# AHHHZ975/SLAM-Duckietown

Measured on AMD Instinct MI355X. Metric: EKF update steps/sec, higher is better.
Workload: dtype f64

## Files before the change

### slam-duckietown_amd/csrc/ekf_kernels.hip

```cpp
#include <algorithm>
#include <type_traits>

#include "ekf_device.h"

#include "ekf_devfn.h"
#include "ekf_host_plan.h"
#include "ekf_launch.h"

namespace ekf {

constexpr int PCS = CMAX + 2;
constexpr int RCH = 8;
constexpr int CPAD = (CMAX + RCH - 1) / RCH * RCH;
constexpr int WCS = KTOT + 1;

constexpr int SQ = (CMAX + 2) / 3;
struct StageRegs {
  double wv[SQ], vv[SQ];
};
__device__ __forceinline__ void stage_issue(StageRegs& R, __amdgpu_buffer_rsrc_t rsV, __amdgpu_buffer_rsrc_t rsW,
                                            int Cl, int c, int kb, int kofs, int ld, int wave, int lane) {
  const int kc = min(kofs + lane, kb - 1);
  const unsigned kW = (unsigned)(((kc >> 2) * (ld >> 4)) * 64 + (kc & 3) * 16) * 8u;
  const unsigned kV = (unsigned)(kc * ld) * 8u;
// ... 1187 lines not shown
  int cmax = Cl;
#pragma unroll
  for (int sh = 32; sh > 0; sh >>= 1) cmax = max(cmax, __shfl_xor(cmax, sh));
  const int kb = kbase;
  const PanelIdx t = panel_idx(P, V, W, mu_in, mu_out, ld, pstride, b, n, w0);
  if (w0 >= neff_eff) {
    if (wave == 0) panel_beyond_bound<MCAP>(t, kb);
    return;
  }
  if (tid < CC + 1) S.sC[tid] = Cl;
  if (kb > 0) {
    const __amdgpu_buffer_rsrc_t rsV = rs_rsrc(t.Vb), rsW = rs_rsrc(t.Wb);
    constexpr int Q = (CC + 3) / 4;
    const int k8 = (kb + 7) & ~7;
    for (int kofs = 0; kofs < kb; kofs += 64) {
      const int k = kofs + lane, kc = min(k, kb - 1);
      const unsigned kW = (unsigned)(((kc >> 2) * (ld >> 4)) * 64 + (kc & 3) * 16) * 8u;
      const unsigned kV = (unsigned)(kc * ld) * 8u;
      double wv[Q], vv[Q];
#pragma unroll
      for (int q = 0; q < Q; ++q) {
        const int a = wave + 4 * q;
        wv[q] = 0.0;
        vv[q] = 0.0;
        if (a < c) {
          const int row = __builtin_amdgcn_readlane(Cl, a);
          wv[q] = ldb8(rsW, kW, (unsigned)((row >> 4) * 64 + (row & 15)) * 8u);
          vv[q] = ldb8(rsV, kV, (unsigned)row * 8u);
        }
      }
#pragma unroll
      for (int q = 0; q < Q; ++q) {
        const int a = wave + 4 * q;
        if (a < CC && k < k8) {
          const bool live = a < c && k < kb;
          S.sF[0][a][k] = live ? wv[q] : 0.0;
          S.sF[1][a][k] = live ? vv[q] : 0.0;
        }
      }
    }
  }
  double X[CC];
  if (wave == 0) {
    int Crow[CC];
#pragma unroll
    for (int a = 0; a < CC; ++a) Crow[a] = __builtin_amdgcn_readlane(Cl, a);
    panel_base_gather<CC>(t, Crow, X);
  } else {
#pragma unroll
    for (int a = 0; a < CC; ++a) X[a] = 0.0;
  }
  __syncthreads();
  if (kb > 0) {
    const double* vlane = t.Vb + t.ii;
    const double* wlane = t.Wb + (long)(t.ii >> 4) * 64 + (t.ii & 15);
    auto gather_pending = [&](auto need_w_tag) {
      constexpr bool NEEDW = decltype(need_w_tag)::value;
      double v[8], w[8];
      pg_load<NEEDW>(vlane, wlane, ld, t.ld16, kb, 8 * wave, v, w);
      for (int k0 = 8 * wave; k0 < kb; k0 += 32) {
        double vn[8], wn[8];
        pg_load<NEEDW>(vlane, wlane, ld, t.ld16, kb, k0 + 32, vn, wn);
        pg_accumulate<CC>(X, v, w, S.sF, S.sC, k0, w0, t.ii);
#pragma unroll
        for (int u = 0; u < 8; ++u) {
          v[u] = vn[u];
          w[u] = wn[u];
        }
      }
    };
    if (cmax > w0) gather_pending(std::true_type{});
    else gather_pending(std::false_type{});
    if (wave > 0) {
#pragma unroll
      for (int a = 0; a < CC; ++a) SP.sPart[wave - 1][a][lane] = X[a];
    }
    __syncthreads();
    if (wave > 0) return;
#pragma unroll
    for (int a = 0; a < CC; ++a) {
      double x = X[a];
#pragma unroll
      for (int q = 0; q < 3; ++q) x += SP.sPart[q][a][lane];
      X[a] = x;
    }
  } else if (wave > 0) {
    return;
  }
  {
    unsigned got = 0;
    for (int spin = 0; spin < SPLIT_SPIN_LIMIT; ++spin) {
      got = __hip_atomic_load(ready + b, __ATOMIC_RELAXED, __HIP_MEMORY_SCOPE_AGENT);
      if (got == seq) break;
      __builtin_amdgcn_s_sleep(4);
    }
    if (got != seq) {
      if (lane == 0) atomicOr(flags + b, EKF_FLAG_INTERNAL);
      return;
    }
    __builtin_amdgcn_fence(__ATOMIC_ACQUIRE, "agent");
  }
  const SolveOut& o = out[b];
  {
    const double2* src = reinterpret_cast<const double2*>(o.it);
    double2* dst = reinterpret_cast<double2*>(S.sIt);
    constexpr int PER = (int)(sizeof(SolveIter) / 16), CNT = MCAP * PER, Q = (CNT + 63) / 64;
    const int count = m * PER;
    double2 t0[Q];
#pragma unroll
    for (int q = 0; q < Q; ++q) t0[q] = src[min(lane + q * 64, CNT - 1)];
#pragma unroll
    for (int q = 0; q < Q; ++q)
      if (lane + q * 64 < count) dst[lane + q * 64] = t0[q];
  }
  WAVE_LDS_SYNC();
  panels_finish<MCAP>(t, o, S.sIt, S.sC, X);
}

template <bool NT>
__device__ __forceinline__ double2 ld2(const double* a) {
  double2 r;
  if (NT) {
    r.x = __builtin_nontemporal_load(a);
    r.y = __builtin_nontemporal_load(a + 1);
  } else {
    r = *reinterpret_cast<const double2*>(a);
  }
  return r;
}
template <bool NT>
__device__ __forceinline__ void st2(double* a, double2 v) {
  if (NT) {
    __builtin_nontemporal_store(v.x, a);
    __builtin_nontemporal_store(v.y, a + 1);
  } else {
    *reinterpret_cast<double2*>(a) = v;
  }
}

constexpr int FTS = 80;

template <int NKTM, int NKL, bool NT>
__global__ __launch_bounds__(256, 2) void k_flush(double* __restrict__ P, const double* __restrict__ V,
                                                  const double* __restrict__ W,
                                                  const double* __restrict__ dacc,
                                                  const int* __restrict__ nact,
                                                  const SolveOut* __restrict__ so, int ld, long pstride,
                                                  int nkt, int rows_per_block, int gx) {
  __shared__ double tiles[4][16 * FTS];
  __shared__ double vlds[NKL > 0 ? 4 : 1][NKL > 0 ? NKL * 4 * 64 : 1];
  const int b = blockIdx.z;
  const int n = min(nact[b], so[b].neff);
  const int wave = __builtin_amdgcn_readfirstlane(threadIdx.x >> 6);
  const int lane = threadIdx.x & 63;
  int bx, by = 0;
  {
    const int total = gridDim.x;
    const int lin = blockIdx.x;
    const int q = total >> 3, r = total & 7, xcd = lin & 7, slot = lin >> 3;
    int rem = ((xcd < r) ? xcd * (q + 1) : r * (q + 1) + (xcd - r) * q) + slot;
    for (;; ++by) {
      const int cnt = gx - (by * rows_per_block) / 256;
      if (rem < cnt || cnt <= 0) break;
      rem -= cnt;
    }
    bx = (by * rows_per_block) / 256 + rem;
  }
  const int j0 = (bx * 4 + wave) * 64;
  const int i_begin = by * rows_per_block;
  const int i_lim = min(n, j0 + 64);
  if (j0 >= n || i_begin >= i_lim) return;
  const int i_end = min(i_lim, i_begin + rows_per_block);
  const int li = lane & 15, lq = lane >> 4;
  const int rr = lane >> 5, rc = (lane & 31) * 2;
  const int ld16 = ld >> 4;
  double* Pb = P + (long)b * pstride;
  const double* Vb = V + (long)b * KTOT * ld;
  const double* Wb = W + (long)b * KTOT * ld;
  double* T = tiles[wave];
  int nct = (n - j0 + 15) >> 4;
  if (nct > 4) nct = 4;

  double vf[NKTM][4];
#pragma unroll
  for (int t = 0; t < NKTM; ++t)
#pragma unroll
    for (int ct = 0; ct < 4; ++ct)
      vf[t][ct] = (t < nkt && ct < nct) ? Vb[(long)(4 * t + lq) * ld + j0 + ct * 16 + li] : 0.0;
  double* VL = vlds[NKL > 0 ? wave : 0];
  if (NKL > 0) {
    double tmp[NKL > 0 ? NKL * 4 : 1];
#pragma unroll
    for (int t = 0; t < NKL; ++t)
#pragma unroll
      for (int ct = 0; ct < 4; ++ct)
        tmp[t * 4 + ct] = Vb[(long)(4 * min(NKTM + t, nkt - 1) + lq) * ld + j0 + ct * 16 + li];
#pragma unroll
    for (int t = 0; t < NKL; ++t)
#pragma unroll
      for (int ct = 0; ct < 4; ++ct) VL[(t * 4 + ct) * 64 + lane] = (NKTM + t < nkt && ct < nct) ? tmp[t * 4 + ct] : 0.0;
    WAVE_SYNC();
  }

  double2 g[8];
  const int lds = p_lds(ld);
  double* Pj = Pb + p_col(ld, j0 + rc);
  auto gload = [&](int i0) {
#pragma unroll
    for (int q = 0; q < 8; ++q) g[q] = ld2<NT>(Pj + (long)(i0 + 2 * q + rr) * lds);
  };
  gload(i_begin);
  const int i_last = i_begin + ((i_end - 1 - i_begin) & ~15);
  constexpr int NKT_ALL = NKTM + NKL;
  constexpr bool EARLYW = NKTM >= 12;
  double wf[NKT_ALL];
  auto wload = [&](int i0) {
    const double* wsrc = Wb + (long)(i0 >> 4) * 64 + lane;
#pragma unroll
    for (int t = 0; t < NKT_ALL; ++t) wf[t] = wsrc[(long)min(t, nkt - 1) * ld16 * 64];
  };
  if (EARLYW) wload(i_begin);
  for (int i0 = i_begin; i0 < i_end; i0 += 16) {
    const int i_next = min(i0 + 16, i_last);
    if (!EARLYW) wload(i0);
#pragma unroll
    for (int q = 0; q < 8; ++q) *reinterpret_cast<double2*>(&T[(2 * q + rr) * FTS + rc]) = g[q];
    WAVE_SYNC();
    gload(i_next);
    double4_t acc[4];
#pragma unroll
    for (int ct = 0; ct < 4; ++ct)
#pragma unroll
      for (int r = 0; r < 4; ++r) acc[ct][r] = T[(lq + 4 * r) * FTS + ct * 16 + li];
    WAVE_SYNC();
#pragma unroll
    for (int t = 0; t < NKTM; ++t)
      if (t < nkt) {
#pragma unroll
        for (int ct = 0; ct < 4; ++ct)
          acc[ct] = __builtin_amdgcn_mfma_f64_16x16x4f64(wf[t], vf[t][ct], acc[ct], 0, 0, 0);
      }
#pragma unroll
    for (int t = 0; t < NKL; ++t)
      if (NKTM + t < nkt) {
#pragma unroll
        for (int ct = 0; ct < 4; ++ct)
          acc[ct] = __builtin_amdgcn_mfma_f64_16x16x4f64(wf[NKTM + t], VL[(t * 4 + ct) * 64 + lane], acc[ct], 0, 0, 0);
      }
    if (i0 == 0 && j0 == 0) {
#pragma unroll
      for (int r = 0; r < 4; ++r) {
        const int row = lq + 4 * r;
        if (row < 3 && li == row) acc[0][r] += dacc[4 * b + row];
      }
    }
#pragma unroll
    for (int ct = 0; ct < 4; ++ct)
#pragma unroll
      for (int r = 0; r < 4; ++r) T[(lq + 4 * r) * FTS + ct * 16 + li] = acc[ct][r];
    if (EARLYW) wload(i_next);
    WAVE_SYNC();
#pragma unroll
    for (int q = 0; q < 8; ++q) {
      const int row = i0 + 2 * q + rr;
      const double2 o = *reinterpret_cast<const double2*>(&T[(2 * q + rr) * FTS + rc]);
      st2<NT>(Pj + (long)row * lds, o);
    }
    WAVE_SYNC();
  }
}


template <bool NT>
__device__ __forceinline__ double2 ldb16(__amdgpu_buffer_rsrc_t rs, unsigned lane_bytes, unsigned tile_bytes) {
  const uint4v_t v = __builtin_amdgcn_raw_buffer_load_b128(rs, (int)lane_bytes, (int)tile_bytes, NT ? 2 : 0);
  double2 r;
  r.x = __builtin_bit_cast(double, uint2v_t{v.x, v.y});
  r.y = __builtin_bit_cast(double, uint2v_t{v.z, v.w});
  return r;
}
template <bool NT>
__device__ __forceinline__ void stb16(__amdgpu_buffer_rsrc_t rs, unsigned lane_bytes, unsigned tile_bytes, double2 v) {
  {
  const uint2v_t a = __builtin_bit_cast(uint2v_t, v.x), b = __builtin_bit_cast(uint2v_t, v.y);
  const uint4v_t d{a.x, a.y, b.x, b.y};
  __builtin_amdgcn_raw_buffer_store_b128(d, rs, (int)lane_bytes, (int)tile_bytes, NT ? 2 : 0);
  asm volatile("s_nop 1" ::"v"(d) : "memory");
  }
}
#define RS_CBAR() asm volatile("" ::: "memory")

template <int NKT, bool NT, bool PAN, bool WV>
__global__ __launch_bounds__(512, 2) void k_flush_rs(double* __restrict__ P, const double* __restrict__ V,
                                                     const double* __restrict__ W,
                                                     const double* __restrict__ dacc,
                                                     const int* __restrict__ nact,
                                                     const SolveOut* __restrict__ so, int ld, long pstride,
                                                     int nkt, int batch, int nrb, int nch, int cs_arg, int mode,
                                                     unsigned* __restrict__ queue, const int* __restrict__ shares,
                                                     const CadOut* __restrict__ wv) {
  constexpr int RPW = NKT / 2;
  __shared__ __attribute__((aligned(16))) double vbuf[2][NKT * 256];
  __shared__ __attribute__((aligned(16))) double img[8][16 * 64];
  __shared__ int s_unit;
  const int wave = __builtin_amdgcn_readfirstlane(threadIdx.x >> 6);
  const int lane = threadIdx.x & 63;
  const int li = lane & 15, lq = lane >> 4;
  const int rr = lane >> 5, rc = (lane & 31) * 2;
  const int ld16 = ld >> 4;
  const int grp = blockIdx.x & 7;
  double* T = img[wave];
  const int rm_base = rr * 64 + (rc ^ (rr << 4));
  const int cd_even = lq * 64 + li + 16 * (lq & 1), cd_odd = lq * 64 + li + 16 * (1 - (lq & 1));
  auto cd_index = [&](int ct, int reg) { return ((ct & 1) ? cd_odd : cd_even) + 16 * (ct & ~1) + 256 * reg; };
  const int stage_base = ((wave >> 2) * 4 + lq) * 64 + (wave & 3) * 16 + li;
  const unsigned pl8 = (unsigned)(PAN ? p_lds(ld) : ld) * 8u;
  const unsigned loff = (unsigned)rr * pl8 + (unsigned)rc * 8u;
  const unsigned lane8 = (unsigned)lane * 8u;

  bool own_empty = false;
  auto pop = [&]() -> int {
    int found = -1;
    for (int a = 0; a < 8 && found < 0; ++a) {
      const int g2 = (grp + a) & 7;
      const int cnt = rs_queue_count(g2, batch, nrb, nch, mode);
      if (cnt == 0) continue;
      unsigned* head = queue + g2 * RS_QSTRIDE;
      if (a > 0 || own_empty) {
        if (__hip_atomic_load(head, __ATOMIC_RELAXED, __HIP_MEMORY_SCOPE_AGENT) >= (unsigned)cnt) continue;
      }
      const unsigned u = atomicAdd(head, 1u);
      if (u < (unsigned)cnt) found = rs_queue_unit(g2, (int)u, batch, nrb, nch, mode);
      else if (a == 0) own_empty = true;
    }
    return found;
  };
  int piece = 0;
  for (;;) {
    __syncthreads();
    int b, rb, u_start, u_count;
    if (mode == 4) {
      if (piece >= RS_PIECES) return;
      const int* pc = shares + ((long)blockIdx.x * RS_PIECES + piece) * 4;
      ++piece;
      b = pc[0];
      rb = pc[1];
      u_start = pc[2];
      u_count = pc[3];
      if (u_count <= 0) return;
    } else {
      if (threadIdx.x == 0) s_unit = pop();
      __syncthreads();
      const int unit = __builtin_amdgcn_readfirstlane(s_unit);
      if (unit < 0) return;
      const int code = unit & 1023;
      b = (unit >> 10) / nrb;
      rb = (unit >> 10) - b * nrb;
      u_count = code == 1023 ? (1 << 20) : cs_arg;
      u_start = code == 1023 ? 0 : code * cs_arg;
    }
    const int n = min(nact[b], so[b].neff);
    const int i0 = rb * RS_ROWS;
    if (i0 >= n) continue;
    const int j_right = ((n - 1) >> 6) << 6;
    const int S_slab = ((j_right - i0) >> 6) + 1;
    if (u_start >= S_slab) continue;
    const int j_last = j_right - 64 * u_start;
    const int S = min(u_count, S_slab - u_start);
    const bool has_diag = u_start + S == S_slab;
    const int i0w = i0 + 16 * wave;
    const int Sw = (i0w < n) ? ((wave < 4 || !has_diag) ? S : S - 1) : 0;
    double* Pb = P + (long)b * pstride;
    const double* Vb = V + (long)b * KTOT * ld;
    const double* Wb = W + (long)b * KTOT * ld;
    const __amdgpu_buffer_rsrc_t rsV = rs_rsrc(Vb), rsW = rs_rsrc(Wb);
    const unsigned ld8 = (unsigned)ld * 8u;
    const unsigned prow = (unsigned)i0w * pl8;
    const double dd0 = dacc[4 * b], dd1 = dacc[4 * b + 1], dd2 = dacc[4 * b + 2];

    auto stage_load = [&](int t, auto i0_tag, auto cnt_tag, double* vs) {
      constexpr int I0 = decltype(i0_tag)::value, CNT = decltype(cnt_tag)::value;
      const int j = j_last - 64 * min(t, S - 1);
#pragma unroll
      for (int i = 0; i < CNT; ++i) vs[i] = ldb8(rsV, lane8, (unsigned)(wave + 8 * (I0 + i)) * ld8 + (unsigned)j * 8u);
    };
    auto stage_store = [&](double* dst, auto i0_tag, auto cnt_tag, const double* vs) {
      constexpr int I0 = decltype(i0_tag)::value, CNT = decltype(cnt_tag)::value;
      double* d0 = dst + stage_base;
#pragma unroll
      for (int i = 0; i < CNT; ++i) {
        d0[(I0 + i) * 512] = (wave + 8 * (I0 + i) < 4 * nkt) ? vs[i] : 0.0;
      }
    };
    using I0_ = std::integral_constant<int, 0>;
    using IH_ = std::integral_constant<int, RPW / 2>;
    using IR_ = std::integral_constant<int, RPW>;
    auto wg_barrier = [&]() {
      asm volatile("s_waitcnt lgkmcnt(0)" ::: "memory");
      __builtin_amdgcn_s_barrier();
      RS_CBAR();
    };

    if (Sw == 0) {
      double vs[RPW];
      stage_load(0, I0_{}, IR_{}, vs);
      stage_store(vbuf[0], I0_{}, IR_{}, vs);
      wg_barrier();
      for (int t = 0; t < S - 1; ++t) {
        stage_load(t + 1, I0_{}, IR_{}, vs);
        stage_store(vbuf[(t + 1) & 1], I0_{}, IR_{}, vs);
        wg_barrier();
      }
      continue;
    }

    double2 g[8];
    auto tile_off = [&](int t) -> unsigned {
      const unsigned j = (unsigned)(j_last - 64 * t);
      return prow + (PAN ? p_col8(ld, j) : j * 8u);
    };
    auto gload = [&](int t) {
      const bool ok = t < Sw;
      const __amdgpu_buffer_rsrc_t rs = rs_rsrc(ok ? (const void*)Pb : (const void*)so);
      const unsigned off = ok ? tile_off(t) : 0u, ld8d = ok ? pl8 : 0u, loffd = ok ? loff : lane8 * 2u;
#pragma unroll
      for (int q = 0; q < 8; ++q) g[q] = ldb16<NT>(rs, loffd, off + (unsigned)q * 2u * ld8d);
    };
    double4_t accs[2][4];
    double wf[NKT];
    double bf[2][4];

    {
      double vs[RPW];
      stage_load(0, I0_{}, IR_{}, vs);
      gload(0);
      if constexpr (!WV) {
#pragma unroll
        for (int t = 0; t < NKT; ++t) {
          const double x = ldb8(rsW, lane8, ((unsigned)t * ld16 + (unsigned)(i0w >> 4)) * 512u);
          wf[t] = (t < nkt) ? x : 0.0;
        }
      } else {
        const CadOut& oc = wv[b];
        const int nsl = min(oc.nslots, CAD_SLOTS), s0c = CAD_SLOTS - nsl;
        const __amdgpu_buffer_rsrc_t rsR = rs_rsrc(oc.rec);
        const unsigned vlane = (unsigned)(2 * (lq >> 1)) * ld8 + (unsigned)li * 8u;
        const unsigned cpart = (unsigned)(lq & 1) * 8u;
#pragma unroll
        for (int t = 0; t < NKT; ++t) {
          const int sl = 2 * t + (lq >> 1), slot = min(s0c + sl, CAD_SLOTS - 1);
          const unsigned roff = (unsigned)cad_rec_off(slot) * 8u + cpart;
          const unsigned voff = ((unsigned)(4 * t) * (unsigned)ld + (unsigned)i0w) * 8u;
          const double e0 = ldb8(rsV, vlane, voff), e1 = ldb8(rsV, vlane + ld8, voff);
          const double sa = ldb8(rsR, roff, 80u), sb = ldb8(rsR, roff, 96u);
          double w = -__builtin_fma(e0, sa, e1 * sb);
          if (i0w == 0) {
            const double x = ldb8(rsW, lane8, (unsigned)t * ld16 * 512u);
            w = li < 3 ? x : w;
          }
          wf[t] = (t < nkt && sl < nsl) ? w : 0.0;
        }
      }
      stage_store(vbuf[0], I0_{}, IR_{}, vs);
#pragma unroll
      for (int q = 0; q < 8; ++q) *reinterpret_cast<double2*>(&T[rm_base + 128 * q]) = g[q];
      RS_CBAR();
#pragma unroll
      for (int ct = 0; ct < 4; ++ct)
#pragma unroll
        for (int r = 0; r < 4; ++r) accs[0][ct][r] = T[cd_index(ct, r)];
      RS_CBAR();
      gload(1);
      wg_barrier();
#pragma unroll
      for (int ct = 0; ct < 4; ++ct) bf[0][ct] = vbuf[0][ct * 64 + lane];
    }

    auto body = [&](auto first_tag, auto stage_tag, auto par_tag, int t) {
      constexpr bool FIRST = decltype(first_tag)::value, STAGE = decltype(stage_tag)::value;
      constexpr int PAR = decltype(par_tag)::value;
      double4_t (&acc)[4] = accs[PAR];
      double4_t (&accn)[4] = accs[1 - PAR];
      const double* vb = vbuf[t & 1];
      double vs[RPW / 2];
      double2 r[4];
      constexpr int NE = FIRST ? 0 : 4, NV = STAGE ? 1 : 0;
      constexpr int OVA = 0, OW0 = OVA + NV, OE1A = OW0 + NE, OE2A = OE1A + NE, OE1B = OE2A + NE, OE2B = OE1B + NE,
                    OC = OE2B + NE, OVB = OC, ON1 = OVB + NV, ON3 = ON1 + 8, ON2 = ON3 + 8, OWB = ON2 + 16, NSIDE = OWB + NV;
      const __amdgpu_buffer_rsrc_t rsP = rs_rsrc(Pb);
      const unsigned off_prev = tile_off(t - 1);
      const bool ok2 = t + 2 < Sw;
      const __amdgpu_buffer_rsrc_t rs2 = rs_rsrc(ok2 ? (const void*)Pb : (const void*)so);
      const unsigned off2 = ok2 ? tile_off(t + 2) : 0u, ld8d = ok2 ? pl8 : 0u, loffd = ok2 ? loff : lane8 * 2u;
      double* vnext = vbuf[(t + 1) & 1];
      auto side = [&](int o) {
        if constexpr (STAGE) {
          if (o == OVA) stage_load(t + 1, I0_{}, IH_{}, vs);
          if (o == OVB) {
            stage_store(vnext, I0_{}, IH_{}, vs);
            stage_load(t + 1, IH_{}, IH_{}, vs);
          }
          if (o == OWB) stage_store(vnext, IH_{}, IH_{}, vs);
        }
        if constexpr (!FIRST) {
          if (o >= OW0 && o < OE1A) {
            const int ct = o - OW0;
            if (ct == 0) RS_CBAR();
#pragma unroll
            for (int rg = 0; rg < 4; ++rg) T[cd_index(ct, rg)] = accn[ct][rg];
            if (ct == 3) RS_CBAR();
          }
          if (o >= OE1A && o < OE2A) r[o - OE1A] = *reinterpret_cast<const double2*>(&T[rm_base + 128 * (o - OE1A)]);
          if (o >= OE2A && o < OE1B) stb16<NT>(rsP, loff, off_prev + (unsigned)(o - OE2A) * 2u * pl8, r[o - OE2A]);
          if (o >= OE1B && o < OE2B) r[o - OE1B] = *reinterpret_cast<const double2*>(&T[rm_base + 128 * (o - OE1B + 4)]);
          if (o >= OE2B && o < OC) stb16<NT>(rsP, loff, off_prev + (unsigned)(o - OE2B + 4) * 2u * pl8, r[o - OE2B]);
        }
        if (o >= ON1 && o < ON1 + 8) {
          const int q = o - ON1;
          if (q == 0) RS_CBAR();
          *reinterpret_cast<double2*>(&T[rm_base + 128 * q]) = g[q];
          if (q == 7) RS_CBAR();
        } else if (o >= ON2 && o < ON2 + 16) {
          const int e = o - ON2;
          accn[e >> 2][e & 3] = T[cd_index(e >> 2, e & 3)];
          if (e == 15) RS_CBAR();
        } else if (o >= ON3 && o < ON3 + 8) {
          const int q = o - ON3;
          g[q] = ldb16<NT>(rs2, loffd, off2 + (unsigned)q * 2u * ld8d);
        }
      };
#pragma unroll
      for (int kt = 0; kt < NKT; ++kt) {
        if (kt + 1 < NKT) {
#pragma unroll
          for (int ct = 0; ct < 4; ++ct) bf[(kt + 1) & 1][ct] = vb[((kt + 1) * 4 + ct) * 64 + lane];
        } else if (STAGE) {
#pragma unroll
          for (int ct = 0; ct < 4; ++ct) bf[0][ct] = vnext[ct * 64 + lane];
        }
        __builtin_amdgcn_sched_barrier(0);
#pragma unroll
        for (int ct = 0; ct < 4; ++ct)
          acc[ct] = __builtin_amdgcn_mfma_f64_16x16x4f64(wf[kt], bf[kt & 1][ct], acc[ct], 0, 0, 0);
        if (kt == 0) {
          if (NV) side(OVA);
        } else if (kt < NKT - 1) {
#pragma unroll
          for (int o = NV + (kt - 1) * (NSIDE - NV) / (NKT - 2); o < NV + kt * (NSIDE - NV) / (NKT - 2); ++o) side(o);
        }
        if (STAGE && kt == NKT - 2) wg_barrier();
        __builtin_amdgcn_sched_barrier(0);
      }
    };
    auto drain = [&](auto par_tag) {
      constexpr int PAR = decltype(par_tag)::value;
      double4_t (&acc)[4] = accs[PAR];
      if (i0w == 0 && has_diag) {
#pragma unroll
        for (int rg = 0; rg < 4; ++rg) {
          const int row = lq + 4 * rg;
          if (row < 3 && li == row) acc[0][rg] += (row == 0) ? dd0 : ((row == 1) ? dd1 : dd2);
        }
      }
      RS_CBAR();
#pragma unroll
      for (int ct = 0; ct < 4; ++ct)
#pragma unroll
        for (int rg = 0; rg < 4; ++rg) T[cd_index(ct, rg)] = acc[ct][rg];
      RS_CBAR();
      const __amdgpu_buffer_rsrc_t rsP = rs_rsrc(Pb);
      const unsigned off_last = tile_off(Sw - 1);
#pragma unroll
      for (int q = 0; q < 8; ++q) {
        const double2 o = *reinterpret_cast<const double2*>(&T[rm_base + 128 * q]);
        stb16<NT>(rsP, loff, off_last + (unsigned)q * 2u * pl8, o);
      }
      RS_CBAR();
    };
    using T_ = std::true_type;
    using F_ = std::false_type;
    using P0 = std::integral_constant<int, 0>;
    using P1 = std::integral_constant<int, 1>;
    if (S == 1) {
      body(T_{}, F_{}, P0{}, 0);
    } else {
      body(T_{}, T_{}, P0{}, 0);
      int t = 1;
      for (; t + 1 < S - 1; t += 2) {
        body(F_{}, T_{}, P1{}, t);
        body(F_{}, T_{}, P0{}, t + 1);
      }
      if (t < S - 1) {
        body(F_{}, T_{}, P1{}, t);
        ++t;
      }
      if (Sw == S) {
        if ((S - 1) & 1) body(F_{}, F_{}, P1{}, S - 1);
        else body(F_{}, F_{}, P0{}, S - 1);
      }
    }
    if ((Sw - 1) & 1) drain(P1{});
    else drain(P0{});
  }
}

__global__ __launch_bounds__(256) void k_predict_rc(double* __restrict__ P,
                                                    const double* __restrict__ mu_in,
                                                    double* __restrict__ mu_out,
                                                    const int* __restrict__ nact,
                                                    const SolveOut* __restrict__ so, int ld,
                                                    long pstride) {
  const int b = blockIdx.y;
  const int n = nact[b];
  const int j = blockIdx.x * 256 + threadIdx.x;
  if (j >= n) return;
  double* Pb = P + (long)b * pstride;
  const double g0 = so[b].g[0], g1 = so[b].g[1];
  if (j >= 3) {
    mu_out[(long)b * ld + j] = mu_in[(long)b * ld + j];
    if (j >= so[b].neff) return;
    double* pj = Pb + p_col(ld, j);
    const int lds = p_lds(ld);
    const double r2 = pj[2 * (long)lds];
    pj[0] += g0 * r2;
    pj[lds] += g1 * r2;
  } else if (j == 0) {
    double X[3][3], Y[3][3];
    for (int r = 0; r < 3; ++r)
      for (int c = 0; c < 3; ++c) X[r][c] = Pb[p_index(ld, min(r, c), max(r, c))];
    for (int c = 0; c < 3; ++c) {
      X[0][c] += g0 * X[2][c];
      X[1][c] += g1 * X[2][c];
    }
    for (int r = 0; r < 3; ++r) {
      Y[r][0] = X[r][0] + g0 * X[r][2];
      Y[r][1] = X[r][1] + g1 * X[r][2];
      Y[r][2] = X[r][2];
      Y[r][r] += so[b].rd[r];
    }
    for (int r = 0; r < 3; ++r)
      for (int c = r; c < 3; ++c) Pb[p_index(ld, r, c)] = Y[r][c];
  }
}

__global__ __launch_bounds__(256) void k_mirror(double* __restrict__ P, const int* __restrict__ nact, int ld,
                                                long pstride) {
  __shared__ double T[64][65];
  const int b = blockIdx.z;
  const int n = nact[b];
  const int ti = blockIdx.y, tj = blockIdx.x;
  if (tj > ti || ti * 64 >= n) return;
  double* Pb = P + (long)b * pstride;
  const int tx = threadIdx.x & 63, ty = threadIdx.x >> 6;
  for (int r = ty; r < 64; r += 4) {
    const int row = tj * 64 + r, col = ti * 64 + tx;
    T[r][tx] = (row < n && col < n) ? Pb[p_index(ld, row, col)] : 0.0;
  }
  __syncthreads();
  for (int r = ty; r < 64; r += 4) {
    const int row = ti * 64 + r, col = tj * 64 + tx;
    if (row < n && col < n && col < row) Pb[p_index(ld, row, col)] = T[tx][r];
  }
}

__global__ __launch_bounds__(64) void k_associate(const DetIn* __restrict__ det, int* __restrict__ tagmap,
                                                  int* __restrict__ nact, int* __restrict__ neff_dev,
                                                  double* __restrict__ mu, double* __restrict__ P,
                                                  double* __restrict__ V, double* __restrict__ W,
                                                  StepIn* __restrict__ step_out,
                                                  AssocOut* __restrict__ assoc_out,
                                                  unsigned* __restrict__ flags, AssocConfig cfg, int ld,
                                                  long pstride, int n_max, int pending_k, int batch) {
#pragma clang fp contract(off)
  const int b = blockIdx.x, lane = threadIdx.x;
  const DetIn& d = det[b];
  int* tm = tagmap + (long)b * TAGMAX;
  double* mub = mu + (long)b * ld;
  double* Pb = P + (long)b * pstride;
  double* Vb = V + (long)b * KTOT * ld;
  double* Wb = W + (long)b * KTOT * ld;
  __shared__ int s_idx[AMAX], s_tag[AMAX], s_cnt[AMAX];
  __shared__ double s_t[AMAX][3], s_err[AMAX];
  __shared__ int c_id[64], c_lm[64], c_ok[64];
  __shared__ double c_t[64][3], c_e[64];
  const int n_old = nact[b];
  const int nl_old = (n_old - 3) / 2;
  int nl = nl_old, m = 0;
  unsigned bad = 0;
  const int count = min(d.count, DMAX);
  if (lane < AMAX) {
    s_idx[lane] = -1;
    s_tag[lane] = -1;
    s_cnt[lane] = 0;
    s_t[lane][0] = s_t[lane][1] = s_t[lane][2] = 0.0;
    s_err[lane] = 0.0;
  }
  for (int q0 = 0; q0 < count; q0 += 64) {
    const int q = q0 + lane;
    int id = -1, lm = -1, ok = 0;
    double t0 = 0.0, t1 = 0.0, t2 = 0.0, er = 0.0;
    if (q < count) {
      id = d.tag_id[q];
      t0 = d.pose_t[q][0];
      t1 = d.pose_t[q][1];
      t2 = d.pose_t[q][2];
      er = d.pose_err[q];
      if (id < 0 || id >= TAGMAX) ok = 2;
      else {
        bool ign = false;
        for (int u = 0; u < cfg.n_ignore; ++u) ign |= (cfg.ignore[u] == id);
        if (!ign && !(t2 * t2 + t0 * t0 > cfg.gate2)) {
          ok = 1;
          lm = tm[id];
        }
      }
    }
    WAVE_LDS_SYNC();
    c_id[lane] = id;
    c_lm[lane] = lm;
    c_ok[lane] = ok;
    c_t[lane][0] = t0;
    c_t[lane][1] = t1;
    c_t[lane][2] = t2;
    c_e[lane] = er;
    WAVE_LDS_SYNC();
    const int nq = min(64, count - q0);
    for (int u = 0; u < nq; ++u) {
      const int ok_u = c_ok[u];
      if (ok_u == 2) { bad |= EKF_FLAG_ASSOC; continue; }
      if (ok_u == 0) continue;
      const int id_u = c_id[u];
      const unsigned long long hit = __ballot(lane < m && s_tag[lane] == id_u);
      int slot = hit ? __builtin_ctzll(hit) : -1;
      if (slot < 0) {
        if (m >= AMAX) { bad |= EKF_FLAG_ASSOC; continue; }
        int lm_u = c_lm[u];
        if (lm_u < 0) {
          if (3 + 2 * (nl + 1) > n_max) { bad |= EKF_FLAG_ASSOC; continue; }
          lm_u = nl++;
          if (lane == 0) tm[id_u] = lm_u;
        }
        slot = m++;
        if (lane == 0) {
          s_idx[slot] = lm_u;
          s_tag[slot] = id_u;
        }
      }
      if (lane == 0) {
        s_t[slot][0] += c_t[u][0];
        s_t[slot][1] += c_t[u][1];
        s_t[slot][2] += c_t[u][2];
        s_err[slot] += c_e[u];
        s_cnt[slot] += 1;
      }
      WAVE_LDS_SYNC();
    }
  }
  if (bad && lane == 0) atomicOr(&flags[b], bad);
  WAVE_LDS_SYNC();
  const int n_new = 3 + 2 * nl;
  AssocOut& ao = assoc_out[b];
  const double px = mub[0], py = mub[1], pth = mub[2];
  if (lane < AMAX) {
    StepIn& so = step_out[(long)(lane / MMAX) * batch + b];
    const int sl = lane % MMAX;
    if (lane < m) {
      const double k = (double)s_cnt[lane];
      const double t0 = s_t[lane][0] / k, t2 = s_t[lane][2] / k;
      const double xr = t2, yr = -t0;
      const double rng = sqrt(xr * xr + yr * yr);
      const double brg = atan2(yr, xr);
      const double xw = px + rng * cos(brg + pth), yw = py + rng * sin(brg + pth);
      const int lm = s_idx[lane];
      so.idx[sl] = lm;
      so.range[sl] = rng;
      so.bearing[sl] = brg;
      ao.idx[lane] = lm;
      ao.tag_id[lane] = s_tag[lane];
      ao.xw[lane] = xw;
      ao.yw[lane] = yw;
      ao.err[lane] = s_err[lane] / k;
      ao.range[lane] = rng;
      ao.bearing[lane] = brg;
      if (lm >= nl_old) {
        mub[3 + 2 * lm] = xw;
        mub[4 + 2 * lm] = yw;
      }
    } else {
      so.idx[sl] = 0;
      so.range[sl] = 0.0;
      so.bearing[sl] = 0.0;
    }
  }
  const int dn = n_new - n_old;
  const int ld16 = ld >> 4;
  for (long e = lane; e < (long)n_new * dn; e += 64) {
    const int r = (int)(e / dn), q = n_old + (int)(e - (long)r * dn);
    Pb[p_index(ld, r, q)] = (r == q) ? cfg.init_var : 0.0;
    if (r < n_old) Pb[p_index(ld, q, r)] = 0.0;
  }
  for (int e = lane; e < pending_k * dn; e += 64) {
    const int k = e / dn, q = n_old + (e - k * dn);
    Vb[(long)k * ld + q] = 0.0;
    Wb[wm_index(ld16, k, q)] = 0.0;
  }
  if (lane == 0) {
    int bound = neff_dev[b];
    for (int u = 0; u < m; ++u) bound = max(bound, 3 + 2 * (s_idx[u] + 1));
    bound = min(bound, n_new);
    neff_dev[b] = bound;
    nact[b] = n_new;
    StepIn& s0 = step_out[b];
    StepIn& s1 = step_out[(long)batch + b];
    s0.lin = d.lin;
    s0.ang = d.ang;
    s0.m = min(m, MMAX);
    s0.flags = FLAG_PREDICT | FLAG_UPDATE;
    s0.neff = cfg.active_bound ? bound : n_new;
    s0.pad = 0;
    s1.lin = 0.0;
    s1.ang = 0.0;
    s1.m = max(m - MMAX, 0);
    s1.flags = FLAG_UPDATE;
    s1.neff = s0.neff;
    s1.pad = 0;
    ao.m = m;
    ao.n_after = n_new;
  }
}

void launch_associate(hipStream_t st, const BankView& k, const DetIn* det, int* tagmap, int* neff_dev, double* mu, StepIn* step_out,
                      AssocOut* assoc_out, const AssocConfig& cfg, int n_max, int pending_k) {
  hipLaunchKernelGGL(k_associate, dim3(k.batch), dim3(64), 0, st, det, tagmap, k.nact, neff_dev, mu, k.P, k.V, k.W, step_out,
                     assoc_out, k.flags, cfg, k.ld, k.pstride, n_max, pending_k, k.batch);
}

__global__ __launch_bounds__(256) void k_add_landmarks(double* __restrict__ Pb, double* __restrict__ mub,
                                                       int ld, int n_old, int n_new, double var,
                                                       const double* __restrict__ xy) {
  const int k2 = n_new - n_old;
  const long total = (long)n_new * k2;
  for (long e = (long)blockIdx.x * 256 + threadIdx.x; e < total; e += (long)gridDim.x * 256) {
    const int r = (int)(e / k2), q = n_old + (int)(e - (long)r * k2);
    Pb[p_index(ld, r, q)] = (r == q) ? var : 0.0;
    if (r < n_old) Pb[p_index(ld, q, r)] = 0.0;
    if (r == 0) mub[q] = xy[q - n_old];
  }
}

__global__ __launch_bounds__(256) void k_fill_diag(double* __restrict__ Pb, int ld, int n,
                                                   const double* __restrict__ diag) {
  const long total = (long)n * n;
  for (long e = (long)blockIdx.x * 256 + threadIdx.x; e < total; e += (long)gridDim.x * 256) {
    const int r = (int)(e / n), c = (int)(e - (long)r * n);
    Pb[p_index(ld, r, c)] = (r == c) ? diag[r] : 0.0;
  }
}

void launch_solve(hipStream_t st, const BankView& k, const StepBufs& s, const StepArgs& a, const DeviceConfig& cfg) {
  with_flag(cfg.gate_rej != nullptr, [&](auto G) {
    with_flag(cfg.noise != nullptr, [&](auto Z) {
      hipLaunchKernelGGL((k_solve<G.value, Z.value>), dim3(k.batch), dim3(256), 0, st, k.P, k.V, k.W, s.dacc_in, s.dacc_out,
                         s.mu_in, s.mu_out, k.nact, a.in, k.so, k.flags, a.fac, a.neff_floor, k.queue, cfg, k.ld, k.pstride, a.kbase);
    });
  });
}
void launch_panels(hipStream_t st, int mcap, bool latency, const BankView& k, const StepBufs& s, const double* fac, int n_hi) {
  with_mcap(mcap, [&](auto M) {
    with_flag(latency, [&](auto L) {
      hipLaunchKernelGGL((k_panels<M.value, 4, L.value>), dim3((n_hi + (L.value ? 63 : 255)) / (L.value ? 64 : 256), k.batch),
                         dim3(256), 0, st, k.P, k.V, k.W, s.mu_in, s.mu_out, k.nact, k.so, fac, k.ld, k.pstride);
    });
  });
}
void launch_step_split_tp(hipStream_t st, int mcap, const BankView& k, const StepBufs& s, const StepArgs& a,
                          const DeviceConfig& cfg, int n_hi) {
  const dim3 grid(1 + (n_hi + 255) / 256, k.batch);
  SplitArgs sa{s.dacc_in, s.dacc_out, a.in, k.so, k.flags, a.fac, a.neff_floor, k.queue, a.mbox, a.ready, a.seq, a.publish, a.kbase, cfg};
  with_mcap(mcap, [&](auto M) {
    if constexpr (M.value <= 8)
      with_flag(cfg.gate_rej != nullptr, [&](auto G) {
        with_flag(cfg.noise != nullptr, [&](auto Z) {
          hipLaunchKernelGGL((k_panels_split<M.value, G.value, Z.value>), grid, dim3(256), 0, st, k.P, k.V, k.W, s.mu_in, s.mu_out,
                             k.nact, k.ld, k.pstride, sa);
        });
      });
  });
}
void launch_step_split(hipStream_t st, int mcap, const BankView& k, const StepBufs& s, const StepArgs& a, const DeviceConfig& cfg, int n_hi) {
  const dim3 grid(1 + (n_hi + 63) / 64, k.batch);
  with_mcap(mcap, [&](auto M) {
    with_flag(cfg.gate_rej != nullptr, [&](auto G) {
      with_flag(cfg.noise != nullptr, [&](auto Z) {
        hipLaunchKernelGGL((k_step_split<M.value, G.value, Z.value>), grid, dim3(256), 0, st, k.P, k.V, k.W, s.dacc_in, s.dacc_out,
                           s.mu_in, s.mu_out, k.nact, a.in, k.so, k.flags, a.fac, a.neff_floor, k.queue, a.ready, a.seq, a.publish,
                           cfg, k.ld, k.pstride, a.kbase);
      });
    });
  });
}
template <typename F>
static void with_nkt(int nkt, F&& f) {
  if (nkt <= 4) f(std::integral_constant<int, 4>{});
// ... 117 lines not shown
```

Baseline: 185,700.

## Prefetch next work unit during flush to hide queue atomic latency

The persistent flush kernel now issues the atomic pop for its own queue's next unit while the current unit is still being processed, and publishes it to a double-buffered shared slot before the drain. This removes one __syncthreads and the serialized atomic round-trip between units. In the static-share mode (mode 4), the next piece descriptor is loaded ahead as well. Popping ahead adds state-machine complexity around own_empty and work-stealing fallback, and may grab a unit slightly earlier than before.

```diff
diff --git a/slam-duckietown_amd/csrc/ekf_kernels.hip b/slam-duckietown_amd/csrc/ekf_kernels.hip
--- a/slam-duckietown_amd/csrc/ekf_kernels.hip
+++ b/slam-duckietown_amd/csrc/ekf_kernels.hip
@@ -1513,7 +1513,7 @@
   constexpr int RPW = NKT / 2;
   __shared__ __attribute__((aligned(16))) double vbuf[2][NKT * 256];
   __shared__ __attribute__((aligned(16))) double img[8][16 * 64];
-  __shared__ int s_unit;
+  __shared__ int s_unit[2];
   const int wave = __builtin_amdgcn_readfirstlane(threadIdx.x >> 6);
   const int lane = threadIdx.x & 63;
   const int li = lane & 15, lq = lane >> 4;
@@ -1530,9 +1530,10 @@
   const unsigned lane8 = (unsigned)lane * 8u;
 
   bool own_empty = false;
-  auto pop = [&]() -> int {
+  const int cnt_own = mode == 4 ? 0 : rs_queue_count(grp, batch, nrb, nch, mode);
+  auto pop_from = [&](int a0) -> int {
     int found = -1;
-    for (int a = 0; a < 8 && found < 0; ++a) {
+    for (int a = a0; a < 8 && found < 0; ++a) {
       const int g2 = (grp + a) & 7;
       const int cnt = rs_queue_count(g2, batch, nrb, nch, mode);
       if (cnt == 0) continue;
@@ -1546,23 +1547,55 @@
     }
     return found;
   };
+  unsigned u_ahead = 0;
+  int ahead = 0;
+  auto pop_issue = [&]() {
+    if (threadIdx.x == 0 && cnt_own > 0 && !own_empty) {
+      unsigned z = 0;
+      asm volatile("" : "+v"(z));
+      u_ahead = atomicAdd(queue + grp * RS_QSTRIDE + z, 1u);
+    }
+  };
+  auto pop_finish = [&](int slot) {
+    if (threadIdx.x == 0 && cnt_own > 0 && !own_empty) {
+      ahead = 2;
+      if (u_ahead < (unsigned)cnt_own) {
+        s_unit[slot] = rs_queue_unit(grp, (int)u_ahead, batch, nrb, nch, mode);
+        ahead = 1;
+      }
+    }
+  };
+  const int* pc = shares + (long)blockIdx.x * RS_PIECES * 4;
   int piece = 0;
-  for (;;) {
+  int pc_b = 0, pc_rb = 0, pc_start = 0, pc_count = 0;
+  if (mode == 4) {
+    pc_b = pc[0];
+    pc_rb = pc[1];
+    pc_start = pc[2];
+    pc_count = pc[3];
+  }
+  for (int cur = 0;; cur ^= 1) {
+    if (mode != 4 && threadIdx.x == 0 && ahead != 1) {
+      if (ahead == 2) own_empty = true;
+      s_unit[cur] = pop_from(ahead == 2 ? 1 : 0);
+    }
+    ahead = 0;
     __syncthreads();
     int b, rb, u_start, u_count;
     if (mode == 4) {
-      if (piece >= RS_PIECES) return;
-      const int* pc = shares + ((long)blockIdx.x * RS_PIECES + piece) * 4;
+      b = pc_b;
+      rb = pc_rb;
+      u_start = pc_start;
+      u_count = pc_count;
+      if (u_count <= 0) return;
       ++piece;
-      b = pc[0];
-      rb = pc[1];
-      u_start = pc[2];
-      u_count = pc[3];
-      if (u_count <= 0) return;
+      const int* pn = pc + min(piece, RS_PIECES - 1) * 4;
+      pc_b = pn[0];
+      pc_rb = pn[1];
+      pc_start = pn[2];
+      pc_count = piece < RS_PIECES ? pn[3] : 0;
     } else {
-      if (threadIdx.x == 0) s_unit = pop();
-      __syncthreads();
-      const int unit = __builtin_amdgcn_readfirstlane(s_unit);
+      const int unit = __builtin_amdgcn_readfirstlane(s_unit[cur]);
       if (unit < 0) return;
       const int code = unit & 1023;
       b = (unit >> 10) / nrb;
@@ -1578,6 +1611,7 @@
     if (u_start >= S_slab) continue;
     const int j_last = j_right - 64 * u_start;
     const int S = min(u_count, S_slab - u_start);
+    if (mode != 4 && S == 1) pop_issue();
     const bool has_diag = u_start + S == S_slab;
     const int i0w = i0 + 16 * wave;
     const int Sw = (i0w < n) ? ((wave < 4 || !has_diag) ? S : S - 1) : 0;
@@ -1801,6 +1835,7 @@
         body(F_{}, T_{}, P1{}, t);
         body(F_{}, T_{}, P0{}, t + 1);
       }
+      if (mode != 4) pop_issue();
       if (t < S - 1) {
         body(F_{}, T_{}, P1{}, t);
         ++t;
@@ -1810,6 +1845,7 @@
         else body(F_{}, F_{}, P0{}, S - 1);
       }
     }
+    if (mode != 4) pop_finish(cur ^ 1);
     if ((Sw - 1) & 1) drain(P1{});
     else drain(P0{});
   }
```

Result: faster. 189,800 (median of 6 runs) (+2.2%).
